# lixirui142/VidToMe

Measured on AMD Instinct MI355X. Metric: denoising steps/sec, 16-frame 512x512 SD-1.5 chunk, ratio=0.5, higher is better.
Workload: dtype f16 tokens; matching f16-MFMA filter + f32 exact refine (f32-identical indices); attention f16 MFMA with f32 accumulate

## Files before the change

### vidtome_amd/csrc/sort.hip

```cpp
#include "common.h"

namespace {

constexpr int T = 256;
constexpr int WAVES = T / 64;
constexpr int RADIX = 256;
constexpr int PASSES = 4;
static_assert(RADIX == T, "thread d handles digit d");

__device__ __forceinline__ unsigned long long same_digit_lanes(int d, unsigned long long valid) {
    unsigned long long m = valid;
#pragma unroll
    for (int b = 0; b < 8; ++b) {
        const unsigned long long bal = __ballot((d >> b) & 1);
        m &= ((d >> b) & 1) ? bal : ~bal;
    }
    return m;
}

__device__ __forceinline__ uint32_t load_key(const uint64_t *kin, const uint32_t *ksrc, int pass, int64_t i) {
    return pass == 0 ? ~(uint32_t)(kin[i] >> 32) : ksrc[i];
}

struct Geo {
    int64_t n;
    int nseg, tiles_per_seg;
};

__global__ __launch_bounds__(T) void sort_hist_kernel(const uint64_t *__restrict__ best, Geo g, int64_t table_ints,
                                                      int *__restrict__ hist) {
    __shared__ int cnt[RADIX];
    const int tid = threadIdx.x, lane = tid & 63;
    const int seg = blockIdx.x, row = blockIdx.y;
    const uint64_t *kin = best + (int64_t)row * g.n;
    const uint32_t *ksrc = nullptr;
    constexpr int pass = 0, sh = 0;
    cnt[tid] = 0;
#pragma unroll
    for (int p = 1; p < PASSES; ++p)
        hist[p * table_ints + ((int64_t)row * g.nseg + seg) * RADIX + tid] = 0;
    __syncthreads();
    for (int t = 0; t < g.tiles_per_seg; ++t) {
        const int64_t i = ((int64_t)seg * g.tiles_per_seg + t) * T + tid;
        const bool ok = i < g.n;
        const int d = ok ? (int)((load_key(kin, ksrc, pass, i) >> sh) & 255u) : 0;
        const unsigned long long m = same_digit_lanes(d, __ballot(ok));
        if (ok && (m & ((1ull << lane) - 1ull)) == 0) atomicAdd(&cnt[d], __popcll(m));
    }
    __syncthreads();
    hist[((int64_t)row * g.nseg + seg) * RADIX + tid] = cnt[tid];
}

__global__ __launch_bounds__(T) void sort_scatter_kernel(const uint64_t *__restrict__ best,
                                                         const uint32_t *__restrict__ ksrc_all,
                                                         const int32_t *__restrict__ psrc_all,
                                                         uint32_t *__restrict__ kdst_all, int32_t *__restrict__ pdst_all,
                                                         Geo g, int pass, int last, const int *__restrict__ hist,
                                                         int *__restrict__ hist_next) {
    __shared__ uint32_t wcnt[WAVES][RADIX];
    __shared__ int running[RADIX];
    __shared__ int part[RADIX];
    const int tid = threadIdx.x, lane = tid & 63, wave = tid >> 6;
    const int seg = blockIdx.x, row = blockIdx.y;
    const uint64_t *kin = best + (int64_t)row * g.n;
    const uint32_t *ksrc = ksrc_all + (int64_t)row * g.n;
    const int32_t *psrc = psrc_all + (int64_t)row * g.n;
    uint32_t *kdst = kdst_all + (int64_t)row * g.n;
    int32_t *pdst = pdst_all + (int64_t)row * g.n;
    const int sh = pass * 8;
    const int seg_keys = g.tiles_per_seg * T;
    int *hnext = hist_next + (int64_t)row * g.nseg * RADIX;
    const unsigned long long below = (1ull << lane) - 1ull;
    {
        const int *h = hist + (int64_t)row * g.nseg * RADIX + tid;
        int tot = 0, bef = 0;
#pragma unroll 8
        for (int e = 0; e < g.nseg; ++e) {
            const int c = h[e * RADIX];
            tot += c;
            bef += e < seg ? c : 0;
        }
        part[tid] = tot;
        __syncthreads();
        for (int off = 1; off < T; off <<= 1) {
            const int v = tid >= off ? part[tid - off] : 0;
            __syncthreads();
            part[tid] += v;
            __syncthreads();
        }
        running[tid] = part[tid] - tot + bef;
    }
#pragma unroll
    for (int w = 0; w < WAVES; ++w) wcnt[w][tid] = 0xffff0000u;
    __syncthreads();
    for (int t = 0; t < g.tiles_per_seg; ++t) {
        const int64_t i = ((int64_t)seg * g.tiles_per_seg + t) * T + tid;
        const bool ok = i < g.n;
        uint32_t key = 0;
        int32_t id = 0;
        int d = 0;
        if (ok) {
            key = load_key(kin, ksrc, pass, i);
            id = pass == 0 ? (int32_t)i : psrc[i];
            d = (int)((key >> sh) & 255u);
        }
        const unsigned long long m = same_digit_lanes(d, __ballot(ok));
        const uint32_t tag = (uint32_t)t << 16;
        if (ok && (m & below) == 0) wcnt[wave][d] = tag | (uint32_t)__popcll(m);
        __syncthreads();
        if (ok) {
            int pos = running[d] + __popcll(m & below);
#pragma unroll
            for (int w = 0; w < WAVES - 1; ++w) {
                const uint32_t e = wcnt[w][d];
                if (w < wave && (e & 0xffff0000u) == tag) pos += (int)(e & 0xffffu);
            }
            if (!last) {
                kdst[pos] = key;
                atomicAdd(&hnext[(pos / seg_keys) * RADIX + (int)((key >> (sh + 8)) & 255u)], 1);
            }
            pdst[pos] = id;
        }
        __syncthreads();
        {
            int tot = 0;
#pragma unroll
            for (int w = 0; w < WAVES; ++w) {
                const uint32_t e = wcnt[w][tid];
                tot += (e & 0xffff0000u) == tag ? (int)(e & 0xffffu) : 0;
            }
            running[tid] += tot;
        }
        __syncthreads();
    }
}

inline Geo make_geo(int64_t n) {
    Geo g;
    g.n = n;
    const int64_t tiles = vtm::cdiv(n, T);
    int64_t tps = vtm::cdiv(tiles, 64);
    if (tps < 1) tps = 1;
    g.tiles_per_seg = (int)tps;
    g.nseg = (int)vtm::cdiv(tiles, tps);
    return g;
}

inline size_t aligned(size_t v) { return (v + 255) & ~(size_t)255; }

}

VTM_EXPORT size_t vtm_sort_ws_bytes(int64_t rows, int64_t n) {
    if (rows <= 0 || n <= 0) return 0;
    const Geo g = make_geo(n);
    return aligned((size_t)rows * n * 16u) + aligned((size_t)PASSES * rows * RADIX * g.nseg * sizeof(int));
}

VTM_EXPORT int vtm_sort_desc(const uint64_t *best, int64_t rows, int64_t n, int32_t *perm, void *ws,
                             size_t ws_bytes, vtm_stream_t stream) {
    VTM_REQUIRE(best && perm && ws, "vtm_sort_desc: null pointer");
    VTM_REQUIRE(rows > 0 && rows <= 65535 && n >= 0 && n < (1ll << 31), "vtm_sort_desc: bad sizes");
    if (ws_bytes < vtm_sort_ws_bytes(rows, n))
        return vtm::fail(VTM_EWORKSPACE, "vtm_sort_desc: workspace %zu < %zu bytes", ws_bytes,
                         vtm_sort_ws_bytes(rows, n));
    if (n == 0) return VTM_OK;
    hipStream_t s = vtm::as_stream(stream);
    const Geo g = make_geo(n);
    VTM_REQUIRE(g.tiles_per_seg < 0xffff, "vtm_sort_desc: row too long for the tile tag");
    char *w = static_cast<char *>(ws);
    uint32_t *k0 = reinterpret_cast<uint32_t *>(w), *k1 = k0 + rows * n;
    int32_t *p0 = reinterpret_cast<int32_t *>(k1 + rows * n), *p1 = p0 + rows * n;
    int *hist = reinterpret_cast<int *>(w + aligned((size_t)rows * n * 16u));
    const dim3 grid((unsigned)g.nseg, (unsigned)rows), block(T);
    const int64_t table_ints = rows * g.nseg * RADIX;
    hipLaunchKernelGGL(sort_hist_kernel, grid, block, 0, s, best, g, table_ints, hist);
    for (int pass = 0; pass < PASSES; ++pass) {
        const uint32_t *ksrc = (pass & 1) ? k1 : k0;
        const int32_t *psrc = (pass & 1) ? p1 : p0;
        uint32_t *kdst = (pass & 1) ? k0 : k1;
        int32_t *pdst = (pass & 1) ? p0 : p1;
        const int last = pass == PASSES - 1;
        if (last) pdst = perm;
        hipLaunchKernelGGL(sort_scatter_kernel, grid, block, 0, s, best, ksrc, psrc, kdst, pdst, g, pass, last,
                           hist + pass * table_ints, hist + (last ? 0 : pass + 1) * table_ints);
    }
    return vtm::launch_status("vtm_sort_desc");
}
```

Measured before the change: 23.46.

## Use 11-bit radix with three passes and per-wave local scatter in sort

Switches the LSD radix sort from 8-bit digits in four passes to 11-bit digits in three passes, which removes one scatter kernel launch and one full read/write of keys. Each scatter block now uses 512 threads. Every wave pre-counts its own contiguous key range into a private shared histogram, so ranking needs only intra-wave ballots instead of per-tile block barriers and cross-wave tag tables. The cost is larger histograms (2048 bins, plus padding per segment), more shared memory, and a pre-count pass over the keys inside the scatter kernel.

After: 23.60 (median of 2 runs). About the same (+0.6%).

```diff
diff --git a/vidtome_amd/csrc/sort.hip b/vidtome_amd/csrc/sort.hip
--- a/vidtome_amd/csrc/sort.hip
+++ b/vidtome_amd/csrc/sort.hip
@@ -3,15 +3,21 @@
 namespace {
 
 constexpr int T = 256;
-constexpr int WAVES = T / 64;
-constexpr int RADIX = 256;
-constexpr int PASSES = 4;
-static_assert(RADIX == T, "thread d handles digit d");
+constexpr int WAVES = 8;
+constexpr int THREADS = 64 * WAVES;
+constexpr int WG_TILES = THREADS / T;
+constexpr int BITS = 11;
+constexpr int RADIX = 1 << BITS;
+constexpr int PASSES = 3;
+constexpr int ROW = RADIX + 64;
+constexpr int DPT = RADIX / THREADS;
+constexpr int CH = 4;
+static_assert(DPT * THREADS == RADIX && PASSES * BITS >= 32 && WG_TILES * T == THREADS, "geometry");
 
 __device__ __forceinline__ unsigned long long same_digit_lanes(int d, unsigned long long valid) {
     unsigned long long m = valid;
 #pragma unroll
-    for (int b = 0; b < 8; ++b) {
+    for (int b = 0; b < BITS; ++b) {
         const unsigned long long bal = __ballot((d >> b) & 1);
         m &= ((d >> b) & 1) ? bal : ~bal;
     }
@@ -22,44 +28,48 @@
     return pass == 0 ? ~(uint32_t)(kin[i] >> 32) : ksrc[i];
 }
 
+__device__ __forceinline__ int digit_of(uint32_t key, int pass) { return (int)((key >> (pass * BITS)) & (RADIX - 1)); }
+
 struct Geo {
     int64_t n;
-    int nseg, tiles_per_seg;
+    int nseg, steps_log2;
 };
 
-__global__ __launch_bounds__(T) void sort_hist_kernel(const uint64_t *__restrict__ best, Geo g, int64_t table_ints,
-                                                      int *__restrict__ hist) {
+__global__ __launch_bounds__(THREADS) void sort_hist_kernel(const uint64_t *__restrict__ best, Geo g,
+                                                            int64_t table_ints, int *__restrict__ hist) {
     __shared__ int cnt[RADIX];
-    const int tid = threadIdx.x, lane = tid & 63;
+    const int tid = threadIdx.x;
     const int seg = blockIdx.x, row = blockIdx.y;
     const uint64_t *kin = best + (int64_t)row * g.n;
-    const uint32_t *ksrc = nullptr;
-    constexpr int pass = 0, sh = 0;
-    cnt[tid] = 0;
-#pragma unroll
-    for (int p = 1; p < PASSES; ++p)
-        hist[p * table_ints + ((int64_t)row * g.nseg + seg) * RADIX + tid] = 0;
-    __syncthreads();
-    for (int t = 0; t < g.tiles_per_seg; ++t) {
-        const int64_t i = ((int64_t)seg * g.tiles_per_seg + t) * T + tid;
-        const bool ok = i < g.n;
-        const int d = ok ? (int)((load_key(kin, ksrc, pass, i) >> sh) & 255u) : 0;
-        const unsigned long long m = same_digit_lanes(d, __ballot(ok));
-        if (ok && (m & ((1ull << lane) - 1ull)) == 0) atomicAdd(&cnt[d], __popcll(m));
-    }
-    __syncthreads();
-    hist[((int64_t)row * g.nseg + seg) * RADIX + tid] = cnt[tid];
-}
-
-__global__ __launch_bounds__(T) void sort_scatter_kernel(const uint64_t *__restrict__ best,
-                                                         const uint32_t *__restrict__ ksrc_all,
-                                                         const int32_t *__restrict__ psrc_all,
-                                                         uint32_t *__restrict__ kdst_all, int32_t *__restrict__ pdst_all,
-                                                         Geo g, int pass, int last, const int *__restrict__ hist,
-                                                         int *__restrict__ hist_next) {
-    __shared__ uint32_t wcnt[WAVES][RADIX];
-    __shared__ int running[RADIX];
-    __shared__ int part[RADIX];
+    int *mine = hist + ((int64_t)row * g.nseg + seg) * ROW + DPT * tid;
+#pragma unroll
+    for (int j = 0; j < DPT; ++j) {
+        cnt[DPT * tid + j] = 0;
+#pragma unroll
+        for (int p = 1; p < PASSES; ++p) mine[p * table_ints + j] = 0;
+    }
+    __syncthreads();
+    const int64_t i0 = ((int64_t)seg << g.steps_log2) * THREADS + tid;
+    const int steps = 1 << g.steps_log2;
+#pragma unroll 4
+    for (int t = 0; t < steps; ++t) {
+        const int64_t i = i0 + (int64_t)t * THREADS;
+        if (i < g.n) atomicAdd(&cnt[digit_of(load_key(kin, nullptr, 0, i), 0)], 1);
+    }
+    __syncthreads();
+#pragma unroll
+    for (int j = 0; j < DPT; ++j) mine[j] = cnt[DPT * tid + j];
+}
+
+__global__ __launch_bounds__(THREADS) void sort_scatter_kernel(const uint64_t *__restrict__ best,
+                                                               const uint32_t *__restrict__ ksrc_all,
+                                                               const int32_t *__restrict__ psrc_all,
+                                                               uint32_t *__restrict__ kdst_all,
+                                                               int32_t *__restrict__ pdst_all, Geo g, int pass, int last,
+                                                               const int *__restrict__ hist,
+                                                               int *__restrict__ hist_next) {
+    __shared__ int run[WAVES][RADIX];
+    __shared__ int wsum[WAVES];
     const int tid = threadIdx.x, lane = tid & 63, wave = tid >> 6;
     const int seg = blockIdx.x, row = blockIdx.y;
     const uint64_t *kin = best + (int64_t)row * g.n;
@@ -67,71 +77,104 @@
     const int32_t *psrc = psrc_all + (int64_t)row * g.n;
     uint32_t *kdst = kdst_all + (int64_t)row * g.n;
     int32_t *pdst = pdst_all + (int64_t)row * g.n;
-    const int sh = pass * 8;
-    const int seg_keys = g.tiles_per_seg * T;
-    int *hnext = hist_next + (int64_t)row * g.nseg * RADIX;
+    int *hnext = hist_next + (int64_t)row * g.nseg * ROW;
     const unsigned long long below = (1ull << lane) - 1ull;
+    const int steps = 1 << g.steps_log2;
+    const int seg_shift = g.steps_log2 + __builtin_ctz(THREADS);
+    const int64_t i0 = (((int64_t)seg * WAVES + wave) << g.steps_log2) * 64 + lane;
+    int *mine = run[wave];
+    uint32_t key[CH];
+    int32_t id[CH];
+    bool ok[CH];
+#pragma unroll
+    for (int u = 0; u < CH; ++u) {
+        const int64_t i = i0 + (int64_t)u * 64;
+        ok[u] = u < steps && i < g.n;
+        key[u] = ok[u] ? load_key(kin, ksrc, pass, i) : 0u;
+        id[u] = pass == 0 ? (int32_t)i : ok[u] ? psrc[i] : 0;
+    }
+#pragma unroll
+    for (int w = 0; w < WAVES; ++w)
+#pragma unroll
+        for (int j = 0; j < DPT; ++j) run[w][DPT * tid + j] = 0;
+    __syncthreads();
+#pragma unroll
+    for (int u = 0; u < CH; ++u)
+        if (ok[u]) atomicAdd(&mine[digit_of(key[u], pass)], 1);
+#pragma unroll 4
+    for (int t = CH; t < steps; ++t) {
+        const int64_t i = i0 + (int64_t)t * 64;
+        if (i < g.n) atomicAdd(&mine[digit_of(load_key(kin, ksrc, pass, i), pass)], 1);
+    }
+    int tot[DPT], off[DPT];
+#pragma unroll
+    for (int j = 0; j < DPT; ++j) tot[j] = off[j] = 0;
     {
-        const int *h = hist + (int64_t)row * g.nseg * RADIX + tid;
-        int tot = 0, bef = 0;
+        const int *h = hist + (int64_t)row * g.nseg * ROW + DPT * tid;
 #pragma unroll 8
         for (int e = 0; e < g.nseg; ++e) {
-            const int c = h[e * RADIX];
-            tot += c;
-            bef += e < seg ? c : 0;
-        }
-        part[tid] = tot;
+#pragma unroll
+            for (int j = 0; j < DPT; ++j) {
+                const int c = h[e * ROW + j];
+                tot[j] += c;
+                off[j] += e < seg ? c : 0;
+            }
+        }
+        int sum = 0;
+#pragma unroll
+        for (int j = 0; j < DPT; ++j) sum += tot[j];
+        int inc = sum;
+#pragma unroll
+        for (int o = 1; o < 64; o <<= 1) {
+            const int v = __shfl_up(inc, o);
+            if (lane >= o) inc += v;
+        }
+        if (lane == 63) wsum[wave] = inc;
         __syncthreads();
-        for (int off = 1; off < T; off <<= 1) {
-            const int v = tid >= off ? part[tid - off] : 0;
-            __syncthreads();
-            part[tid] += v;
-            __syncthreads();
-        }
-        running[tid] = part[tid] - tot + bef;
-    }
-#pragma unroll
-    for (int w = 0; w < WAVES; ++w) wcnt[w][tid] = 0xffff0000u;
-    __syncthreads();
-    for (int t = 0; t < g.tiles_per_seg; ++t) {
-        const int64_t i = ((int64_t)seg * g.tiles_per_seg + t) * T + tid;
-        const bool ok = i < g.n;
-        uint32_t key = 0;
-        int32_t id = 0;
-        int d = 0;
-        if (ok) {
-            key = load_key(kin, ksrc, pass, i);
-            id = pass == 0 ? (int32_t)i : psrc[i];
-            d = (int)((key >> sh) & 255u);
-        }
-        const unsigned long long m = same_digit_lanes(d, __ballot(ok));
-        const uint32_t tag = (uint32_t)t << 16;
-        if (ok && (m & below) == 0) wcnt[wave][d] = tag | (uint32_t)__popcll(m);
-        __syncthreads();
-        if (ok) {
-            int pos = running[d] + __popcll(m & below);
-#pragma unroll
-            for (int w = 0; w < WAVES - 1; ++w) {
-                const uint32_t e = wcnt[w][d];
-                if (w < wave && (e & 0xffff0000u) == tag) pos += (int)(e & 0xffffu);
+        int before = inc - sum;
+#pragma unroll
+        for (int w = 0; w < WAVES - 1; ++w) before += w < wave ? wsum[w] : 0;
+#pragma unroll
+        for (int j = 0; j < DPT; ++j) {
+            off[j] += before;
+            before += tot[j];
+        }
+    }
+#pragma unroll
+    for (int w = 0; w < WAVES; ++w) {
+#pragma unroll
+        for (int j = 0; j < DPT; ++j) {
+            const int c = run[w][DPT * tid + j];
+            run[w][DPT * tid + j] = off[j];
+            off[j] += c;
+        }
+    }
+    __syncthreads();
+    for (int t0 = 0; t0 < steps; t0 += CH) {
+        if (t0 > 0) {
+#pragma unroll
+            for (int u = 0; u < CH; ++u) {
+                const int64_t i = i0 + (int64_t)(t0 + u) * 64;
+                ok[u] = t0 + u < steps && i < g.n;
+                key[u] = ok[u] ? load_key(kin, ksrc, pass, i) : 0u;
+                id[u] = pass == 0 ? (int32_t)i : ok[u] ? psrc[i] : 0;
             }
-            if (!last) {
-                kdst[pos] = key;
-                atomicAdd(&hnext[(pos / seg_keys) * RADIX + (int)((key >> (sh + 8)) & 255u)], 1);
+        }
+#pragma unroll
+        for (int u = 0; u < CH; ++u) {
+            const int d = ok[u] ? digit_of(key[u], pass) : 0;
+            const unsigned long long m = same_digit_lanes(d, __ballot(ok[u]));
+            if (ok[u]) {
+                const int first = mine[d];
+                const int pos = first + __popcll(m & below);
+                if ((m & below) == 0) mine[d] = first + __popcll(m);
+                if (!last) {
+                    kdst[pos] = key[u];
+                    atomicAdd(&hnext[(pos >> seg_shift) * ROW + digit_of(key[u], pass + 1)], 1);
+                }
+                pdst[pos] = id[u];
             }
-            pdst[pos] = id;
-        }
-        __syncthreads();
-        {
-            int tot = 0;
-#pragma unroll
-            for (int w = 0; w < WAVES; ++w) {
-                const uint32_t e = wcnt[w][tid];
-                tot += (e & 0xffff0000u) == tag ? (int)(e & 0xffffu) : 0;
-            }
-            running[tid] += tot;
-        }
-        __syncthreads();
+        }
     }
 }
 
@@ -140,9 +183,12 @@
     g.n = n;
     const int64_t tiles = vtm::cdiv(n, T);
     int64_t tps = vtm::cdiv(tiles, 64);
-    if (tps < 1) tps = 1;
-    g.tiles_per_seg = (int)tps;
+    int lg = 0;
+    while (((int64_t)WG_TILES << lg) < tps) ++lg;
+    tps = (int64_t)WG_TILES << lg;
+    g.steps_log2 = lg;
     g.nseg = (int)vtm::cdiv(tiles, tps);
+    if (g.nseg < 1) g.nseg = 1;
     return g;
 }
 
@@ -153,7 +199,7 @@
 VTM_EXPORT size_t vtm_sort_ws_bytes(int64_t rows, int64_t n) {
     if (rows <= 0 || n <= 0) return 0;
     const Geo g = make_geo(n);
-    return aligned((size_t)rows * n * 16u) + aligned((size_t)PASSES * rows * RADIX * g.nseg * sizeof(int));
+    return aligned((size_t)rows * n * 16u) + aligned((size_t)PASSES * rows * ROW * g.nseg * sizeof(int));
 }
 
 VTM_EXPORT int vtm_sort_desc(const uint64_t *best, int64_t rows, int64_t n, int32_t *perm, void *ws,
@@ -166,13 +212,12 @@
     if (n == 0) return VTM_OK;
     hipStream_t s = vtm::as_stream(stream);
     const Geo g = make_geo(n);
-    VTM_REQUIRE(g.tiles_per_seg < 0xffff, "vtm_sort_desc: row too long for the tile tag");
     char *w = static_cast<char *>(ws);
     uint32_t *k0 = reinterpret_cast<uint32_t *>(w), *k1 = k0 + rows * n;
     int32_t *p0 = reinterpret_cast<int32_t *>(k1 + rows * n), *p1 = p0 + rows * n;
     int *hist = reinterpret_cast<int *>(w + aligned((size_t)rows * n * 16u));
-    const dim3 grid((unsigned)g.nseg, (unsigned)rows), block(T);
-    const int64_t table_ints = rows * g.nseg * RADIX;
+    const dim3 grid((unsigned)g.nseg, (unsigned)rows), block(THREADS);
+    const int64_t table_ints = rows * g.nseg * ROW;
     hipLaunchKernelGGL(sort_hist_kernel, grid, block, 0, s, best, g, table_ints, hist);
     for (int pass = 0; pass < PASSES; ++pass) {
         const uint32_t *ksrc = (pass & 1) ? k1 : k0;
```
